# sjy-dv/coltt

Measured on AMD Instinct MI355X. Metric: queries/sec @ recall@10, 10Mx768 HNSW, higher is better.
Workload: dtype f32

## Files before the change

coltt_amd/csrc/pq.hip:

```cpp
#include <algorithm>
#include <atomic>
#include <type_traits>

#include "common.hpp"
#include "exact.hpp"
#include "select.hpp"

using namespace coltt;
using namespace coltt::dev;

namespace {

typedef float f32x2 __attribute__((ext_vector_type(2)));
constexpr int PQ_LDS_MAX = 152 * 1024;

template <int KIND, int LEN = 0>
__device__ __forceinline__ float pq_dist(const float* __restrict__ x, const float* __restrict__ y, int len_rt) {
  const int len = LEN > 0 ? LEN : len_rt;
  float acc[32];
#pragma unroll
  for (int u = 0; u < 32; u++) acc[u] = 0.f;
#define PQ_BLOCK_(I_)                                                                                   \
  _Pragma("unroll") for (int u = 0; u < 32; u++) {                                                      \
    const float xv = x[(I_) + u], yv = y[(I_) + u];                                                     \
// ... 121 lines not shown
}

__global__ void pq_place_codes_kernel(const uint8_t* __restrict__ src, uint64_t n, int m, int C, const uint32_t* __restrict__ slots, uint64_t slot_base,
                                      uint8_t* __restrict__ codes, int T, int PB, uint32_t* __restrict__ bad) {
  const uint64_t t = (uint64_t)blockIdx.x * blockDim.x + threadIdx.x;
  if (t >= n * (uint64_t)m) return;
  const uint64_t i = t / m; const int j = (int)(t - i * m);
  const uint8_t c = src[t];
  if ((int)c >= C) { atomicAdd(bad, 1u); return; }
  codes[code_offset(slots ? slots[i] : slot_base + i, j, T, PB)] = c;
}
__global__ void pq_fetch_codes_kernel(const uint8_t* __restrict__ codes, int T, int PB, uint64_t first, uint64_t n, int m, uint8_t* __restrict__ out) {
  const uint64_t t = (uint64_t)blockIdx.x * blockDim.x + threadIdx.x;
  if (t >= n * (uint64_t)m) return;
  const uint64_t i = t / m; const int j = (int)(t - i * m);
  out[t] = codes[code_offset(first + i, j, T, PB)];
}
__global__ void pq_move_row_kernel(uint8_t* __restrict__ codes, int T, int PB, int mp, uint64_t dst, uint64_t src) {
  const int j = (int)(blockIdx.x * blockDim.x + threadIdx.x);
  if (j < mp) codes[code_offset(dst, j, T, PB)] = codes[code_offset(src, j, T, PB)];
}

__global__ void pq_train_init_kernel(const float* __restrict__ vecs, int m, int C, int dsub, float* __restrict__ cb) {
  const uint64_t t = (uint64_t)blockIdx.x * blockDim.x + threadIdx.x;
  if (t >= (uint64_t)m * C * dsub) return;
  const int e = (int)(t % dsub); const int c = (int)((t / dsub) % C); const int j = (int)(t / ((uint64_t)dsub * C));
  cb[t] = vecs[((size_t)c * m + j) * dsub + e];
}
__global__ void pq_train_update_kernel(const float* __restrict__ vecs, uint64_t n, int m, int C, int dsub, const uint8_t* __restrict__ codes,
                                       int T, int PB, float* __restrict__ cb) {
  const uint64_t t = (uint64_t)blockIdx.x * blockDim.x + threadIdx.x;
  if (t >= (uint64_t)m * C * dsub) return;
  const int e = (int)(t % dsub); const int c = (int)((t / dsub) % C); const int j = (int)(t / ((uint64_t)dsub * C));
  float s = 0.f; uint32_t cnt = 0;
  for (uint64_t i = 0; i < n; i++) {
    if (codes[code_offset(i, j, T, PB)] != (uint8_t)c) continue;
    s += vecs[(i * (uint64_t)m + j) * dsub + e];
    cnt++;
  }
  if (cnt) cb[t] = div_rn(s, (float)cnt);
}

template <int W> struct PqRaw;
template <> struct PqRaw<1> { typedef uint32_t type; };
template <> struct PqRaw<2> { typedef u32x2e type; };
template <> struct PqRaw<4> { typedef u32x4e type; };
template <int W> __device__ __forceinline__ uint32_t pq_word(const typename PqRaw<W>::type& r, int i) {
  if constexpr (W == 1) return r;
  else if constexpr (W == 2) return i == 0 ? r.x : r.y;
  else return i == 0 ? r.x : (i == 1 ? r.y : (i == 2 ? r.z : r.w));
}

constexpr int PQ_RING = 8;

template <int W, int QB>
__global__ __launch_bounds__(1024) void pq_scan_kernel(const uint8_t* __restrict__ codes, int T, int mp, const float* __restrict__ lut_g, int nq,
                                                       uint64_t begin, uint64_t end, const uint32_t* __restrict__ thr,
                                                       unsigned long long* __restrict__ cand, uint32_t* __restrict__ cnt, uint32_t cap) {
  extern __shared__ __attribute__((aligned(16))) float lut[];
  typedef typename PqRaw<W>::type raw_t;
  const int tid = threadIdx.x, lane = tid & 63;
  const int q0 = (int)blockIdx.y * QB;
  const size_t lq = (size_t)mp * 256;
  if constexpr (QB == 1) {
    const f32x4* src = reinterpret_cast<const f32x4*>(lut_g + (size_t)q0 * lq);
    f32x4* dst = reinterpret_cast<f32x4*>(lut);
    for (int i = tid; i < mp * 64; i += blockDim.x) dst[i] = src[i];
  } else if constexpr (QB == 2) {
    for (int i = tid; i < mp * 256; i += blockDim.x) {
      f32x2 v;
      v.x = lut_g[(size_t)q0 * lq + i];
      v.y = q0 + 1 < nq ? lut_g[(size_t)(q0 + 1) * lq + i] : 0.f;
      reinterpret_cast<f32x2*>(lut)[i] = v;
    }
  } else {
    for (int i = tid; i < mp * 256; i += blockDim.x) {
      f32x4 v;
      v.x = lut_g[(size_t)q0 * lq + i];
      v.y = q0 + 1 < nq ? lut_g[(size_t)(q0 + 1) * lq + i] : 0.f;
      v.z = q0 + 2 < nq ? lut_g[(size_t)(q0 + 2) * lq + i] : 0.f;
      v.w = q0 + 3 < nq ? lut_g[(size_t)(q0 + 3) * lq + i] : 0.f;
      reinterpret_cast<f32x4*>(lut)[i] = v;
    }
  }
  uint32_t th[QB]; bool qv[QB];
#pragma unroll
  for (int q = 0; q < QB; q++) { qv[q] = q0 + q < nq; th[q] = qv[q] ? thr[q0 + q] : 0u; }
  __syncthreads();

  const int wave = __builtin_amdgcn_readfirstlane(tid >> 6);
  const int wpb = (int)(blockDim.x >> 6);
  const uint64_t tile_end = (end + 63) >> 6;
  const uint64_t tstride = (uint64_t)gridDim.x * wpb;
  uint64_t ptile = (begin >> 6) + (uint64_t)blockIdx.x * wpb + wave, ctile = ptile;
  int pt = 0, ct = 0;
  if (ctile >= tile_end) return;
  constexpr int PBYTES = 4 * W;
#define PQ_LOAD(dst)                                                                                                      \
  {                                                                                                                       \
    const uint64_t lt_ = ptile < tile_end ? ptile : tile_end - 1;                                                         \
    dst = *reinterpret_cast<const raw_t*>(codes + ((lt_ * (uint64_t)T + (uint64_t)pt) * 64 + (uint64_t)lane) * PBYTES);   \
    if (++pt == T) { pt = 0; ptile += tstride; }                                                                          \
  }
  constexpr int R = W == 4 ? PQ_RING : 2 * PQ_RING;
  raw_t cur[R], nxt[R];
#pragma unroll
  for (int u = 0; u < R; u++) PQ_LOAD(cur[u])
  typedef typename std::conditional<QB == 1, float, typename std::conditional<QB == 2, f32x2, f32x4>::type>::type acc_t;
  acc_t acc;
  if constexpr (QB == 1) acc = 0.f; else if constexpr (QB == 2) acc = f32x2{0.f, 0.f}; else acc = f32x4{0.f, 0.f, 0.f, 0.f};
  while (ctile < tile_end) {
#pragma unroll
    for (int u = 0; u < R; u++) PQ_LOAD(nxt[u])
#pragma unroll
    for (int u = 0; u < R; u++) {
      const raw_t raw = cur[u];
      const float* lp = lut + (size_t)ct * (PBYTES * 256 * QB);
#pragma unroll
      for (int d = 0; d < W; d++) {
        const uint32_t wd = pq_word<W>(raw, d);
#pragma unroll
        for (int b = 0; b < 4; b++) {
          const uint32_t code = (wd >> (8 * b)) & 0xffu;
          if constexpr (QB == 1) acc = acc + lp[(d * 4 + b) * 256 + code];
          else if constexpr (QB == 2) acc = acc + *reinterpret_cast<const f32x2*>(lp + ((size_t)(d * 4 + b) * 256 + code) * 2);
          else acc = acc + *reinterpret_cast<const f32x4*>(lp + ((size_t)(d * 4 + b) * 256 + code) * 4);
        }
      }
      if (++ct == T) {
        const uint64_t row = (ctile << 6) + (uint64_t)lane;
        const bool valid = ctile < tile_end && row >= begin && row < end;
#pragma unroll
        for (int q = 0; q < QB; q++) {
          float sc;
          if constexpr (QB == 1) sc = acc; else if constexpr (QB == 2) sc = q == 0 ? acc.x : acc.y; else sc = q == 0 ? acc.x : (q == 1 ? acc.y : (q == 2 ? acc.z : acc.w));
          const uint32_t key = score_key(sc);
          if (valid && qv[q] && key <= th[q]) {
            const uint32_t idx = atomicAdd(&cnt[q0 + q], 1u);
            if (idx < cap) cand[(size_t)(q0 + q) * cap + idx] = ((unsigned long long)key << 32) | (uint32_t)row;
          }
        }
        if constexpr (QB == 1) acc = 0.f; else if constexpr (QB == 2) acc = f32x2{0.f, 0.f}; else acc = f32x4{0.f, 0.f, 0.f, 0.f};
        ct = 0; ctile += tstride;
      }
    }
#pragma unroll
    for (int u = 0; u < R; u++) cur[u] = nxt[u];
  }
#undef PQ_LOAD
}

constexpr uint32_t PQ1_KMAX = 64;
constexpr uint32_t PQ1_WL = 128;
static __device__ __forceinline__ void pq_wave_sync() {
  __builtin_amdgcn_fence(__ATOMIC_RELEASE, "wavefront");
  __builtin_amdgcn_wave_barrier();
  __builtin_amdgcn_fence(__ATOMIC_ACQUIRE, "wavefront");
}
static __device__ __forceinline__ uint32_t pq1_compress(unsigned long long* __restrict__ wl, uint32_t nl, uint32_t k, uint32_t& thw, int lane, uint32_t* __restrict__ ovf) {
  const bool h0 = (uint32_t)lane < nl, h1 = 64u + (uint32_t)lane < nl;
  const unsigned long long e0 = h0 ? wl[lane] : ~0ull, e1 = h1 ? wl[64 + lane] : ~0ull;
  uint32_t r0 = 0, r1 = 0;
  for (uint32_t j = 0; j < nl; j++) { const unsigned long long ej = wl[j]; r0 += ej < e0 ? 1u : 0u; r1 += ej < e1 ? 1u : 0u; }
  const unsigned long long m0 = __ballot(h0 && r0 == k - 1), m1 = __ballot(h1 && r1 == k - 1);
  const uint32_t kth = m0 ? (uint32_t)__builtin_amdgcn_readlane((int)(uint32_t)(e0 >> 32), __builtin_ctzll(m0))
                          : (uint32_t)__builtin_amdgcn_readlane((int)(uint32_t)(e1 >> 32), __builtin_ctzll(m1 | (1ull << 63)));
  const bool k0 = h0 && (uint32_t)(e0 >> 32) <= kth, k1 = h1 && (uint32_t)(e1 >> 32) <= kth;
  const unsigned long long b0 = __ballot(k0), b1 = __ballot(k1), lt = (1ull << lane) - 1ull;
  const uint32_t n0 = (uint32_t)__popcll(b0), p1 = n0 + (uint32_t)__popcll(b1 & lt), tot = n0 + (uint32_t)__popcll(b1);
  pq_wave_sync();
  if (k0) wl[__popcll(b0 & lt)] = e0;
  if (k1 && p1 < PQ1_WL) wl[p1] = e1;
  pq_wave_sync();
  thw = kth;
  if (tot > 64u) { if (lane == 0) atomicOr(ovf, 1u); return 64u; }
  return tot;
}

template <int W>
__global__ __launch_bounds__(1024) void pq_scan1_kernel(const uint8_t* __restrict__ codes, int T, int mp, const float* __restrict__ lut_g, uint64_t end, uint32_t k,
                                                        unsigned long long* __restrict__ cand, uint32_t* __restrict__ cnt, uint32_t cap, uint32_t* __restrict__ ovf) {
  extern __shared__ __attribute__((aligned(16))) float lut[];
  __shared__ uint32_t s_wn[16], s_kth;
  typedef typename PqRaw<W>::type raw_t;
  const int tid = threadIdx.x, lane = tid & 63;
  const int wave = __builtin_amdgcn_readfirstlane(tid >> 6);
  const int wpb = (int)(blockDim.x >> 6);
  unsigned long long* const wl = reinterpret_cast<unsigned long long*>(lut + (size_t)mp * 256) + (size_t)wave * PQ1_WL;
  unsigned long long* const bl = reinterpret_cast<unsigned long long*>(lut + (size_t)mp * 256) + (size_t)wpb * PQ1_WL;
  {
    const f32x4* src = reinterpret_cast<const f32x4*>(lut_g);
    f32x4* dst = reinterpret_cast<f32x4*>(lut);
    for (int i = tid; i < mp * 64; i += blockDim.x) dst[i] = src[i];
  }
  if (tid == 0) s_kth = 0xffffffffu;
  __syncthreads();
  const uint64_t tile_end = (end + 63) >> 6;
  const uint64_t tstride = (uint64_t)gridDim.x * wpb;
  uint64_t ptile = (uint64_t)blockIdx.x * wpb + wave, ctile = ptile;
  int pt = 0, ct = 0;
  uint32_t nl = 0, thw = 0xffffffffu;
  const unsigned long long ltm = (1ull << lane) - 1ull;
  constexpr int PBYTES = 4 * W;
#define PQ_LOAD(dst)                                                                                                      \
  {                                                                                                                       \
    const uint64_t lt_ = ptile < tile_end ? ptile : tile_end - 1;                                                         \
    dst = *reinterpret_cast<const raw_t*>(codes + ((lt_ * (uint64_t)T + (uint64_t)pt) * 64 + (uint64_t)lane) * PBYTES);   \
    if (++pt == T) { pt = 0; ptile += tstride; }                                                                          \
  }
  constexpr int R = W == 4 ? PQ_RING : 2 * PQ_RING;
  if (ctile < tile_end) {
    raw_t cur[R], nxt[R];
#pragma unroll
    for (int u = 0; u < R; u++) PQ_LOAD(cur[u])
    float acc = 0.f;
    while (ctile < tile_end) {
#pragma unroll
      for (int u = 0; u < R; u++) PQ_LOAD(nxt[u])
#pragma unroll
      for (int u = 0; u < R; u++) {
        const raw_t raw = cur[u];
        const float* lp = lut + (size_t)ct * (PBYTES * 256);
#pragma unroll
        for (int d = 0; d < W; d++) {
          const uint32_t wd = pq_word<W>(raw, d);
#pragma unroll
          for (int b = 0; b < 4; b++) acc = acc + lp[(d * 4 + b) * 256 + ((wd >> (8 * b)) & 0xffu)];
        }
        if (++ct == T) {
          const uint64_t row = (ctile << 6) + (uint64_t)lane;
          const uint32_t key = score_key(acc);
          const bool pass = ctile < tile_end && row < end && key <= thw;
          const unsigned long long pm = __ballot(pass);
          if (pm) {
            if (pass) wl[nl + (uint32_t)__popcll(pm & ltm)] = ((unsigned long long)key << 32) | (uint32_t)row;
            nl += (uint32_t)__popcll(pm);
            pq_wave_sync();
            if (nl > 64u) nl = pq1_compress(wl, nl, k, thw, lane, ovf);
          }
          acc = 0.f; ct = 0; ctile += tstride;
        }
      }
#pragma unroll
      for (int u = 0; u < R; u++) cur[u] = nxt[u];
    }
    if (nl > k) nl = pq1_compress(wl, nl, k, thw, lane, ovf);
  }
#undef PQ_LOAD
  if (lane == 0) s_wn[wave] = nl;
  __syncthreads();
  uint32_t base = 0, tot = 0;
  for (int w = 0; w < wpb; w++) { const uint32_t c = s_wn[w]; base += w < wave ? c : 0u; tot += c; }
  for (uint32_t i = lane; i < nl; i += 64) bl[base + i] = wl[i];
  __syncthreads();
  if (tot >= k) {
    for (uint32_t i = tid; i < tot; i += blockDim.x) {
      const unsigned long long e = bl[i];
      uint32_t rank = 0;
      for (uint32_t j = 0; j < tot; j++) rank += bl[j] < e ? 1u : 0u;
      if (rank == k - 1) s_kth = (uint32_t)(e >> 32);
    }
    __syncthreads();
  }
  const uint32_t kth = s_kth;
  for (uint32_t i = tid; i < tot; i += blockDim.x) {
    const unsigned long long e = bl[i];
    if ((uint32_t)(e >> 32) > kth) continue;
    const uint32_t idx = atomicAdd(&cnt[0], 1u);
    if (idx < cap) cand[idx] = e;
  }
}

__global__ __launch_bounds__(256) void pq_scan_global_kernel(const uint8_t* __restrict__ codes, int T, int PB, int m, int mp, const float* __restrict__ lut_g,
                                                             uint64_t begin, uint64_t end, const uint32_t* __restrict__ thr,
                                                             unsigned long long* __restrict__ cand, uint32_t* __restrict__ cnt, uint32_t cap) {
  const int q = blockIdx.y;
  const float* lut = lut_g + (size_t)q * mp * 256;
  const uint32_t th = thr[q];
  for (uint64_t row = begin + (uint64_t)blockIdx.x * blockDim.x + threadIdx.x; row < end; row += (uint64_t)gridDim.x * blockDim.x) {
    float acc = 0.f;
    for (int j = 0; j < m; j++) acc = acc + lut[(size_t)j * 256 + codes[code_offset(row, j, T, PB)]];
    const uint32_t key = score_key(acc);
    if (key <= th) {
      const uint32_t idx = atomicAdd(&cnt[q], 1u);
      if (idx < cap) cand[(size_t)q * cap + idx] = ((unsigned long long)key << 32) | (uint32_t)row;
    }
  }
}

__global__ void pq_init_kernel(uint32_t* cnt, uint32_t* thr, uint32_t* ovf, int nq) {
  const int q = blockIdx.x * blockDim.x + threadIdx.x;
  if (q < nq) { cnt[q] = 0; thr[q] = 0xffffffffu; }
  if (q == 0) *ovf = 0;
}

struct PCtx {
  hipStream_t stream = nullptr;
  hipEvent_t ev0 = nullptr, ev1 = nullptr, evs0 = nullptr, evs1 = nullptr;
  DevBuf w_q, w_lut, w_cand, w_cnt, w_out_ids, w_out_sc, w_out_cnt;
  int init() {
    COLTT_HIP(hipStreamCreateWithFlags(&stream, hipStreamNonBlocking));
    COLTT_HIP(hipEventCreate(&ev0)); COLTT_HIP(hipEventCreate(&ev1));
    COLTT_HIP(hipEventCreate(&evs0)); COLTT_HIP(hipEventCreate(&evs1));
    return COLTT_OK;
  }
  ~PCtx() {
    for (hipEvent_t e : {ev0, ev1, evs0, evs1}) if (e) (void)hipEventDestroy(e);
    if (stream) (void)hipStreamDestroy(stream);
  }
};

struct Pq : Object {
  uint32_t dim = 0, m = 0, C = 0, dsub = 0; int metric = 0;
  int mp = 0, PB = 0, T = 0;
  bool trained = false;
  uint64_t n = 0, cap = 0;
  DevBuf cb, codes, ids;
  bool dense = true; uint64_t dense_base = 0;
  std::unordered_map<uint64_t, uint32_t> id2slot; std::vector<uint64_t> h_ids;
  hipStream_t stream = nullptr;
  DevBuf w_raw, w_slots, w_bad;
  std::atomic<float> last_ms{0.f}, last_scan_ms{0.f};
  std::atomic<uint64_t> last_scan_rows{0};
  CtxPool<PCtx> pool;
  ~Pq() override { (void)hipSetDevice(device); if (stream) (void)hipStreamDestroy(stream); }
  size_t tile_bytes() const { return (size_t)64 * mp; }
  int reserve(uint64_t rows) {
    if (rows <= cap) return COLTT_OK;
    uint64_t nc = std::max<uint64_t>({rows, cap + cap / 2, 1024});
    nc = (nc + 63) & ~63ull;
    const size_t old = codes.cap;
    COLTT_TRY(codes.reserve(nc / 64 * tile_bytes(), true, stream));
    if (codes.cap > old) {
      COLTT_HIP(hipMemsetAsync(codes.as<uint8_t>() + old, 0, codes.cap - old, stream));
      COLTT_HIP(hipStreamSynchronize(stream));
    }
    if (!dense) COLTT_TRY(ids.reserve(nc * 8, true, stream));
    cap = nc;
    return COLTT_OK;
  }
  int undense() {
    if (!dense) return COLTT_OK;
    h_ids.resize(n); id2slot.reserve(n * 2);
    for (uint64_t s = 0; s < n; s++) { h_ids[s] = dense_base + s; id2slot[dense_base + s] = (uint32_t)s; }
    dense = false;
    COLTT_TRY(ids.reserve(std::max<uint64_t>(cap, 1024) * 8, false, stream));
    if (n) COLTT_HIP(hipMemcpyAsync(ids.p, h_ids.data(), n * 8, hipMemcpyHostToDevice, stream));
    COLTT_HIP(hipStreamSynchronize(stream));
    return COLTT_OK;
  }
};

struct PqPlan { std::vector<uint32_t> slots; std::vector<uint64_t> new_ids; uint64_t nn = 0; };
int plan_upsert(const Pq* p, const uint64_t* ids, uint64_t first_id, size_t n, PqPlan& pl) {
  pl.slots.resize(n); pl.nn = p->n;
  std::unordered_map<uint64_t, uint32_t> fresh;
  for (size_t i = 0; i < n; i++) {
    const uint64_t id = ids ? ids[i] : first_id + i;
    auto it = p->id2slot.find(id);
    if (it != p->id2slot.end()) { pl.slots[i] = it->second; continue; }
    auto r = fresh.emplace(id, (uint32_t)pl.nn);
    if (r.second) { pl.new_ids.push_back(id); pl.nn++; }
    pl.slots[i] = r.first->second;
  }
  if (pl.nn > 0xffffffffull) return fail(COLTT_E_UNSUPPORTED, "pq upsert: more than 2^32-1 rows in one store");
  return COLTT_OK;
}
void last_wins(const PqPlan& pl, size_t n, std::vector<size_t>& keep) {
  std::unordered_map<uint32_t, size_t> last;
  for (size_t i = 0; i < n; i++) last[pl.slots[i]] = i;
  keep.clear();
  if (last.size() == n) return;
  for (size_t i = 0; i < n; i++) if (last[pl.slots[i]] == i) keep.push_back(i);
}
void commit_upsert(Pq* p, const PqPlan& pl) {
  for (size_t j = 0; j < pl.new_ids.size(); j++) { p->id2slot[pl.new_ids[j]] = (uint32_t)(p->n + j); p->h_ids.push_back(pl.new_ids[j]); }
  p->n = pl.nn;
}

int launch_encode(Pq* p, hipStream_t s, const float* d_vecs, uint64_t n, const uint32_t* d_slots, uint64_t slot_base, uint8_t* codes) {
  if (n == 0) return COLTT_OK;
  const size_t cb_bytes = (size_t)p->C * p->dsub * 4;
  const int lds_cb = cb_bytes <= 64 * 1024;
  const size_t lds = lds_cb ? cb_bytes : 0;
  dim3 grid(ceil_div(n, 256), p->m);
#define PQ_ENC(DS)                                                                                                               \
  {                                                                                                                              \
    auto kern = pq_encode_kernel<DS>;                                                                                            \
    if (lds > 48 * 1024) COLTT_HIP(hipFuncSetAttribute(reinterpret_cast<const void*>(kern), hipFuncAttributeMaxDynamicSharedMemorySize, (int)lds)); \
    kern<<<grid, 256, lds, s>>>(p->cb.as<float>(), (int)p->m, (int)p->C, (int)p->dsub, d_vecs, n, d_slots, slot_base, lds_cb, codes, p->T, p->PB); \
  }
  switch (p->dsub) {
    case 4: PQ_ENC(4) break;
    case 8: PQ_ENC(8) break;
    case 12: PQ_ENC(12) break;
    case 16: PQ_ENC(16) break;
    case 24: PQ_ENC(24) break;
    case 32: PQ_ENC(32) break;
    default: PQ_ENC(0) break;
  }
#undef PQ_ENC
  COLTT_HIP(hipGetLastError());
  return COLTT_OK;
}

template <int W>
int launch_scan_w(Pq* p, PCtx* c, int QBq, uint64_t b, uint64_t e, int nq, const float* lut, const uint32_t* thr, unsigned long long* cand, uint32_t* cnt, uint32_t cap) {
  const size_t lds = (size_t)p->mp * 1024 * QBq;
  const int threads = lds > 80 * 1024 ? 1024 : (lds > 40 * 1024 ? 512 : 256);
  const int wpb = threads / 64;
  const int blocks_per_cu = std::max<int>(1, std::min<int>(2048 / threads, (int)((160 * 1024) / std::max<size_t>(lds, 1))));
  const uint64_t tiles = ((e + 63) >> 6) - (b >> 6);
  const uint32_t gx = (uint32_t)std::max<uint64_t>(1, std::min<uint64_t>((tiles + wpb - 1) / wpb, (uint64_t)256 * blocks_per_cu));
  dim3 grid(gx, (nq + QBq - 1) / QBq);
  if (QBq == 1) {
    auto kern = pq_scan_kernel<W, 1>;
    COLTT_HIP(hipFuncSetAttribute(reinterpret_cast<const void*>(kern), hipFuncAttributeMaxDynamicSharedMemorySize, (int)std::max<size_t>(lds, 1024)));
    kern<<<grid, threads, lds, c->stream>>>(p->codes.as<uint8_t>(), p->T, p->mp, lut, nq, b, e, thr, cand, cnt, cap);
  } else if (QBq == 2) {
    auto kern = pq_scan_kernel<W, 2>;
    COLTT_HIP(hipFuncSetAttribute(reinterpret_cast<const void*>(kern), hipFuncAttributeMaxDynamicSharedMemorySize, (int)std::max<size_t>(lds, 1024)));
    kern<<<grid, threads, lds, c->stream>>>(p->codes.as<uint8_t>(), p->T, p->mp, lut, nq, b, e, thr, cand, cnt, cap);
  } else {
    auto kern = pq_scan_kernel<W, 4>;
    COLTT_HIP(hipFuncSetAttribute(reinterpret_cast<const void*>(kern), hipFuncAttributeMaxDynamicSharedMemorySize, (int)std::max<size_t>(lds, 1024)));
    kern<<<grid, threads, lds, c->stream>>>(p->codes.as<uint8_t>(), p->T, p->mp, lut, nq, b, e, thr, cand, cnt, cap);
  }
  COLTT_HIP(hipGetLastError());
  return COLTT_OK;
}

int launch_scan(Pq* p, PCtx* c, uint64_t b, uint64_t e, int nq, const float* lut, const uint32_t* thr, unsigned long long* cand, uint32_t* cnt, uint32_t cap) {
  const size_t one = (size_t)p->mp * 1024;
  if (one > (size_t)PQ_LDS_MAX) {
    dim3 grid((uint32_t)std::min<uint64_t>(ceil_div(e - b, 256), 256 * 8), nq);
    pq_scan_global_kernel<<<grid, 256, 0, c->stream>>>(p->codes.as<uint8_t>(), p->T, p->PB, (int)p->m, p->mp, lut, b, e, thr, cand, cnt, cap);
    COLTT_HIP(hipGetLastError());
    return COLTT_OK;
  }
  const int QBq = nq < 2 ? 1 : (one * 4 <= (size_t)PQ_LDS_MAX ? 4 : (one * 2 <= (size_t)PQ_LDS_MAX ? 2 : 1));
  if (p->PB == 16) return launch_scan_w<4>(p, c, QBq, b, e, nq, lut, thr, cand, cnt, cap);
  if (p->PB == 8) return launch_scan_w<2>(p, c, QBq, b, e, nq, lut, thr, cand, cnt, cap);
  return launch_scan_w<1>(p, c, QBq, b, e, nq, lut, thr, cand, cnt, cap);
}

bool scan1_geometry(const Pq* p, uint32_t k, int* threads_out, size_t* lds_out) {
  const char* e = getenv("COLTT_PQ_ONE");
  const bool off = e && e[0] == '0';
  if (off || k > PQ1_KMAX) return false;
  const size_t table = (size_t)p->mp * 1024;
  const int threads = table > 80 * 1024 ? 1024 : (table > 40 * 1024 ? 512 : 256);
  const size_t lds = table + (size_t)(threads / 64) * (PQ1_WL + 64) * 8;
  if (lds > (size_t)PQ_LDS_MAX) return false;
  *threads_out = threads; *lds_out = lds;
  return true;
}
template <int W>
int launch_scan1_w(Pq* p, PCtx* c, int threads, size_t lds, uint64_t total, uint32_t k, const float* lut, unsigned long long* cand, uint32_t* cnt, uint32_t cap, uint32_t* ovf) {
  const int wpb = threads / 64;
  const int blocks_per_cu = std::max<int>(1, std::min<int>(2048 / threads, (int)((160 * 1024) / lds)));
  const uint64_t tiles = (total + 63) >> 6;
  const uint32_t gx = (uint32_t)std::max<uint64_t>(1, std::min<uint64_t>((tiles + wpb - 1) / wpb, (uint64_t)256 * blocks_per_cu));
  auto kern = pq_scan1_kernel<W>;
  COLTT_HIP(hipFuncSetAttribute(reinterpret_cast<const void*>(kern), hipFuncAttributeMaxDynamicSharedMemorySize, (int)lds));
  kern<<<gx, threads, lds, c->stream>>>(p->codes.as<uint8_t>(), p->T, p->mp, lut, total, k, cand, cnt, cap, ovf);
  COLTT_HIP(hipGetLastError());
  return COLTT_OK;
}

constexpr size_t PQ_GROUP = 256;
int pq_search_group(Pq* p, PCtx* c, const float* queries, bool q_on_device, size_t nq, uint32_t k, uint64_t* out_ids, float* out_scores,
                    uint32_t* out_counts, bool out_on_device, float* acc_ms) {
  const float* d_q = queries;
  if (!q_on_device) {
    COLTT_TRY(c->w_q.reserve(nq * p->dim * 4));
    COLTT_HIP(hipMemcpyAsync(c->w_q.p, queries, nq * p->dim * 4, hipMemcpyHostToDevice, c->stream));
    d_q = c->w_q.as<float>();
  }
  uint64_t* d_oi = out_ids; float* d_os = out_scores; uint32_t* d_oc = out_counts;
  if (!out_on_device) {
    COLTT_TRY(c->w_out_ids.reserve(nq * k * 8)); COLTT_TRY(c->w_out_sc.reserve(nq * k * 4)); COLTT_TRY(c->w_out_cnt.reserve(nq * 4));
    d_oi = c->w_out_ids.as<uint64_t>(); d_os = c->w_out_sc.as<float>(); d_oc = c->w_out_cnt.as<uint32_t>();
  }
  const uint32_t cap = std::max<uint32_t>(65536u, 8u * k);
  COLTT_TRY(c->w_lut.reserve(nq * (size_t)p->mp * 256 * 4));
  COLTT_TRY(c->w_cand.reserve(nq * (size_t)cap * 8));
  COLTT_TRY(c->w_cnt.reserve((2 * nq + 4) * 4));
  uint32_t* cnt = c->w_cnt.as<uint32_t>(); uint32_t* thr = cnt + nq; uint32_t* ovf = thr + nq;
  unsigned long long* cand = c->w_cand.as<unsigned long long>();
  float* lut = c->w_lut.as<float>();
  const uint64_t* ids = p->dense ? nullptr : p->ids.as<uint64_t>();
  const uint64_t total = p->n;
  COLTT_HIP(hipEventRecord(c->ev0, c->stream));
  {
    dim3 grid(p->mp, (uint32_t)nq);
    if (p->metric == COLTT_PQ_COSINE) pq_lut_kernel<0><<<grid, 256, 0, c->stream>>>(p->cb.as<float>(), (int)p->m, (int)p->C, (int)p->dsub, d_q, p->mp, lut, cnt, thr, ovf);
    else if (p->metric == COLTT_PQ_EUCLIDEAN) pq_lut_kernel<1><<<grid, 256, 0, c->stream>>>(p->cb.as<float>(), (int)p->m, (int)p->C, (int)p->dsub, d_q, p->mp, lut, cnt, thr, ovf);
    else pq_lut_kernel<2><<<grid, 256, 0, c->stream>>>(p->cb.as<float>(), (int)p->m, (int)p->C, (int)p->dsub, d_q, p->mp, lut, cnt, thr, ovf);
  }
  bool timed_scan = false;
  auto scan = [&](uint64_t b, uint64_t e, bool big) -> int {
    if (big) COLTT_HIP(hipEventRecord(c->evs0, c->stream));
    COLTT_TRY(launch_scan(p, c, b, e, (int)nq, lut, thr, cand, cnt, cap));
    if (big) { COLTT_HIP(hipEventRecord(c->evs1, c->stream)); timed_scan = true; p->last_scan_rows.store(e - b); }
    flat_select_kernel<<<(uint32_t)nq, 256, 0, c->stream>>>(cand, cnt, thr, cap, k, 1, ids, p->dense_base, ovf, d_oi, d_os, d_oc);
    return COLTT_OK;
  };
  int t1 = 0; size_t lds1 = 0;
  if (total == 0) {
    flat_select_kernel<<<(uint32_t)nq, 256, 0, c->stream>>>(cand, cnt, thr, cap, k, 1, ids, p->dense_base, ovf, d_oi, d_os, d_oc);
  } else if (nq == 1 && total > 65536 && scan1_geometry(p, k, &t1, &lds1)) {
    COLTT_HIP(hipEventRecord(c->evs0, c->stream));
    if (p->PB == 16) COLTT_TRY(launch_scan1_w<4>(p, c, t1, lds1, total, k, lut, cand, cnt, cap, ovf));
    else if (p->PB == 8) COLTT_TRY(launch_scan1_w<2>(p, c, t1, lds1, total, k, lut, cand, cnt, cap, ovf));
    else COLTT_TRY(launch_scan1_w<1>(p, c, t1, lds1, total, k, lut, cand, cnt, cap, ovf));
    COLTT_HIP(hipEventRecord(c->evs1, c->stream)); timed_scan = true; p->last_scan_rows.store(total);
    flat_select_kernel<<<1, 256, 0, c->stream>>>(cand, cnt, thr, cap, k, 1, ids, p->dense_base, ovf, d_oi, d_os, d_oc);
  } else {
    uint64_t s0 = std::min<uint64_t>({total, (uint64_t)cap, (std::max<uint64_t>(4096, 4ull * k) + 63) & ~63ull});
    for (uint64_t b = 0, e = s0; b < total; b = e, e = std::min<uint64_t>(total, e * 64)) COLTT_TRY(scan(b, e, e == total));
  }
  auto fetch = [&](uint32_t* h_ovf) -> int {
    COLTT_HIP(hipEventRecord(c->ev1, c->stream));
    COLTT_HIP(hipGetLastError());
    COLTT_HIP(hipMemcpyAsync(h_ovf, ovf, 4, hipMemcpyDeviceToHost, c->stream));
    if (!out_on_device) {
      COLTT_HIP(hipMemcpyAsync(out_ids, d_oi, nq * k * 8, hipMemcpyDeviceToHost, c->stream));
      COLTT_HIP(hipMemcpyAsync(out_scores, d_os, nq * k * 4, hipMemcpyDeviceToHost, c->stream));
      COLTT_HIP(hipMemcpyAsync(out_counts, d_oc, nq * 4, hipMemcpyDeviceToHost, c->stream));
    }
    COLTT_HIP(hipStreamSynchronize(c->stream));
    return COLTT_OK;
  };
  uint32_t h_ovf = 0;
  COLTT_TRY(fetch(&h_ovf));
  if (h_ovf && total) {
    pq_init_kernel<<<ceil_div(nq, 256), 256, 0, c->stream>>>(cnt, thr, ovf, (int)nq);
    const uint64_t seg = (cap - std::min<uint32_t>(k, cap / 2)) & ~63ull;
    for (uint64_t b = 0; b < total; b += seg) COLTT_TRY(scan(b, std::min<uint64_t>(total, b + seg), false));
    COLTT_TRY(fetch(&h_ovf));
  }
  float ms = 0.f;
  (void)hipEventElapsedTime(&ms, c->ev0, c->ev1);
  if (acc_ms) *acc_ms += ms;
  if (timed_scan) { float sms = 0.f; (void)hipEventElapsedTime(&sms, c->evs0, c->evs1); p->last_scan_ms.store(sms); }
  return COLTT_OK;
}

int pq_search_common(Pq* p, PCtx* c, const float* queries, bool q_on_device, size_t nq, uint32_t k, uint64_t* out_ids, float* out_scores,
                     uint32_t* out_counts, bool out_on_device) {
  if (k == 0 || k > K_MAX) return fail(COLTT_E_UNSUPPORTED, "pq search: k=%u outside [1,%u]", k, K_MAX);
  if (nq == 0) return COLTT_OK;
  if (!p->trained) return fail(COLTT_E_INVALID, "pq search: the quantiser has no codebooks yet (coltt_pq_set_codebooks / coltt_pq_train)");
  float total_ms = 0.f;
  for (size_t q0 = 0; q0 < nq; q0 += PQ_GROUP) {
    const size_t gn = std::min(PQ_GROUP, nq - q0);
    COLTT_TRY(pq_search_group(p, c, queries + q0 * p->dim, q_on_device, gn, k, out_ids + q0 * k, out_scores + q0 * k, out_counts + q0, out_on_device, &total_ms));
  }
  p->last_ms.store(total_ms);
  return COLTT_OK;
}

}

int coltt::pq_snapshot(coltt_handle_t h, PqShape* shape, DevBuf* cb_out, hipStream_t s) {
  auto p = lookup<Pq>(h);
  if (!p) return fail(COLTT_E_NOT_FOUND, "pq snapshot: unknown quantiser handle");
  ReadLock g(p->rw);
  if (!p->trained) return fail(COLTT_E_INVALID, "pq snapshot: the quantiser has no codebooks yet (coltt_pq_set_codebooks / coltt_pq_train)");
  shape->dim = p->dim; shape->m = p->m; shape->C = p->C; shape->dsub = p->dsub; shape->metric = p->metric;
  const size_t bytes = (size_t)p->m * p->C * p->dsub * 4;
  COLTT_TRY(cb_out->reserve(bytes));
  COLTT_HIP(hipMemcpyAsync(cb_out->p, p->cb.p, bytes, hipMemcpyDefault, s));
  COLTT_HIP(hipStreamSynchronize(s));
  return COLTT_OK;
}

int coltt::pq_encode_rowmajor(hipStream_t s, const float* d_cb, const PqShape& sh, const float* d_vecs, uint64_t n, uint8_t* d_codes, uint32_t row_bytes) {
  if (n == 0) return COLTT_OK;
  const size_t cb_bytes = (size_t)sh.C * sh.dsub * 4;
  const int lds_cb = cb_bytes <= 64 * 1024;
  const size_t lds = lds_cb ? cb_bytes : 0;
  dim3 grid(ceil_div(n, 256), sh.m);
#define PQ_ENC(DS)                                                                                                               \
  {                                                                                                                              \
    auto kern = pq_encode_kernel<DS>;                                                                                            \
    if (lds > 48 * 1024) COLTT_HIP(hipFuncSetAttribute(reinterpret_cast<const void*>(kern), hipFuncAttributeMaxDynamicSharedMemorySize, (int)lds)); \
    kern<<<grid, 256, lds, s>>>(d_cb, (int)sh.m, (int)sh.C, (int)sh.dsub, d_vecs, n, nullptr, 0, lds_cb, d_codes, 1, (int)row_bytes);    \
  }
  switch (sh.dsub) {
    case 4: PQ_ENC(4) break;
    case 8: PQ_ENC(8) break;
    case 12: PQ_ENC(12) break;
    case 16: PQ_ENC(16) break;
    case 24: PQ_ENC(24) break;
    case 32: PQ_ENC(32) break;
    default: PQ_ENC(0) break;
  }
#undef PQ_ENC
  COLTT_HIP(hipGetLastError());
  return COLTT_OK;
}

int coltt::pq_lut16_batch(hipStream_t s, const float* d_cb, const PqShape& sh, const float* d_queries, size_t nq, uint32_t mp, uint32_t shift, uint32_t* d_qmax, unsigned short* d_lut) {
  if (nq == 0) return COLTT_OK;
  if (shift < 4 || shift > 8 || (1u << shift) < sh.C) return fail(COLTT_E_INVALID, "pq_lut16: %u centroids do not fit rows of %u entries", sh.C, 1u << shift);
  dim3 grid(ceil_div(mp, 256u >> shift), (uint32_t)nq);
  COLTT_HIP(hipMemsetAsync(d_qmax, 0, nq * 4, s));
#define COLTT_L16(K)                                                                                                                        \
  do {                                                                                                                                      \
    pq_lut16_max_kernel<K><<<grid, 256, 0, s>>>(d_cb, (int)sh.m, (int)sh.C, (int)sh.dsub, d_queries, (int)mp, (int)shift, d_qmax);          \
    pq_lut16_kernel<K><<<grid, 256, 0, s>>>(d_cb, (int)sh.m, (int)sh.C, (int)sh.dsub, d_queries, (int)mp, (int)shift, d_qmax, d_lut);        \
  } while (0)
  if (sh.metric == COLTT_PQ_COSINE) COLTT_L16(0);
  else if (sh.metric == COLTT_PQ_EUCLIDEAN) COLTT_L16(1);
  else COLTT_L16(2);
#undef COLTT_L16
  COLTT_HIP(hipGetLastError());
  return COLTT_OK;
}
int coltt::pq_centroid_norm_max(hipStream_t s, const float* d_cb, const PqShape& sh, uint32_t* d_scratch, float* out) {
  COLTT_HIP(hipMemsetAsync(d_scratch, 0, 4, s));
  const uint32_t nc = sh.m * sh.C;
  pq_centroid_norm_max_kernel<<<ceil_div(nc, 256u), 256, 0, s>>>(d_cb, nc, (int)sh.dsub, d_scratch);
  COLTT_HIP(hipGetLastError());
  uint32_t bits = 0;
  COLTT_HIP(hipMemcpyAsync(&bits, d_scratch, 4, hipMemcpyDeviceToHost, s));
  COLTT_HIP(hipStreamSynchronize(s));
  std::memcpy(out, &bits, 4);
  return COLTT_OK;
}

extern "C" {

int coltt_pq_create(uint32_t dim, int metric, uint32_t num_subvectors, uint32_t num_centroids, coltt_handle_t* out) {
  if (!out) return fail(COLTT_E_INVALID, "pq_create: out is NULL");
  if (metric != COLTT_PQ_COSINE && metric != COLTT_PQ_EUCLIDEAN && metric != COLTT_PQ_DOT) return fail(COLTT_E_INVALID, "pq_create: bad metric %d", metric);
  if (num_centroids < 2 || num_centroids > 256) return fail(COLTT_E_INVALID, "pq_create: numCentroids %u outside [2,256]", num_centroids);
  if (num_subvectors < 2) return fail(COLTT_E_INVALID, "pq_create: numSubVectors %u < 2", num_subvectors);
  if (dim == 0 || dim % num_subvectors) return fail(COLTT_E_INVALID, "pq_create: dim %u is not a multiple of numSubVectors %u", dim, num_subvectors);
  if (num_subvectors > 4096) return fail(COLTT_E_UNSUPPORTED, "pq_create: numSubVectors %u > 4096", num_subvectors);
  COLTT_DEVICE(-1);
  auto p = std::make_shared<Pq>();
  p->dim = dim; p->metric = metric; p->m = num_subvectors; p->C = num_centroids; p->dsub = dim / num_subvectors;
  p->mp = (int)((num_subvectors + 3) & ~3u);
  p->PB = p->mp % 16 == 0 ? 16 : (p->mp % 8 == 0 ? 8 : 4);
  p->T = p->mp / p->PB;
  p->device = coltt_dev_scope_.device();
  COLTT_HIP(hipStreamCreateWithFlags(&p->stream, hipStreamNonBlocking));
  COLTT_TRY(p->cb.reserve((size_t)p->m * p->C * p->dsub * 4));
  COLTT_TRY(p->w_bad.reserve(16));
  *out = Registry::get().add(p);
  return COLTT_OK;
}

int coltt_pq_destroy(coltt_handle_t h) {
  if (!Registry::get().erase(h)) return fail(COLTT_E_NOT_FOUND, "pq_destroy: unknown handle");
  return COLTT_OK;
}

int coltt_pq_set_codebooks(coltt_handle_t h, const float* codebooks) {
  auto p = lookup<Pq>(h);
  if (!p) return fail(COLTT_E_NOT_FOUND, "pq_set_codebooks: unknown handle");
  if (!codebooks) return fail(COLTT_E_INVALID, "pq_set_codebooks: NULL codebooks");
  WriteLock g(p->rw);
  COLTT_DEVICE(p->device);
  if (p->n) return fail(COLTT_E_INVALID, "pq_set_codebooks: the store holds %llu encoded rows — their codes belong to the current codebooks", (unsigned long long)p->n);
  COLTT_HIP(hipMemcpyAsync(p->cb.p, codebooks, (size_t)p->m * p->C * p->dsub * 4, hipMemcpyHostToDevice, p->stream));
  COLTT_HIP(hipStreamSynchronize(p->stream));
  p->trained = true;
// ... 254 lines not shown
```

coltt_amd/csrc/select.hpp:

```cpp
#pragma once
#include "exact.hpp"

namespace coltt {
namespace dev {

constexpr uint32_t K_MAX = 2048;
constexpr uint32_t SELECT_SMALL = 512;

static __device__ __forceinline__ uint64_t slot_id(const uint64_t* ids, uint64_t dense_base, uint32_t slot) {
  return ids ? ids[slot] : dense_base + slot;
}

typedef uint32_t sel_u32x4 __attribute__((ext_vector_type(4)));
typedef unsigned long long sel_u64x2 __attribute__((ext_vector_type(2)));
static __device__ __forceinline__ uint32_t sel_rank(const uint32_t* __restrict__ keys, const uint64_t* __restrict__ ids, uint32_t n4, uint32_t ki, uint64_t ii) {
  uint32_t rank = 0;
  for (uint32_t j = 0; j < n4; j += 4) {
    const sel_u32x4 kj = *reinterpret_cast<const sel_u32x4*>(keys + j);
    const sel_u64x2 ia = *reinterpret_cast<const sel_u64x2*>(ids + j), ib = *reinterpret_cast<const sel_u64x2*>(ids + j + 2);
    rank += ((kj.x < ki) || (kj.x == ki && ia.x < ii)) ? 1u : 0u;
    rank += ((kj.y < ki) || (kj.y == ki && ia.y < ii)) ? 1u : 0u;
    rank += ((kj.z < ki) || (kj.z == ki && ib.x < ii)) ? 1u : 0u;
    rank += ((kj.w < ki) || (kj.w == ki && ib.y < ii)) ? 1u : 0u;
  }
  return rank;
}

static __device__ __forceinline__ void sel_find_digit(const uint32_t* __restrict__ hist, uint32_t need, uint32_t* __restrict__ wave_tot,
                                                      uint32_t* __restrict__ s_digit, uint32_t* __restrict__ s_need) {
  const int tid = threadIdx.x, lane = tid & 63, wave = tid >> 6;
  const uint32_t h = hist[tid];
  uint32_t inc = h;
#pragma unroll
  for (int d = 1; d < 64; d <<= 1) {
    const uint32_t up = (uint32_t)__shfl_up((int)inc, d, 64);
    if (lane >= d) inc += up;
  }
  if (lane == 63) wave_tot[wave] = inc;
  __syncthreads();
  uint32_t base = 0;
  for (int w = 0; w < wave; w++) base += wave_tot[w];
  inc += base;
  const uint32_t exc = inc - h;
  if (exc < need && need <= inc) { *s_digit = (uint32_t)tid; *s_need = need - exc; }
}

template <uint32_t KCAP = K_MAX>
static __device__ __forceinline__ void flat_select_block(
    const int q, unsigned long long* __restrict__ cand_all, uint32_t* __restrict__ cnt_all, uint32_t* __restrict__ thr_all,
    uint32_t cap, uint32_t k, int nearest, const uint64_t* __restrict__ ids, uint64_t dense_base,
    uint32_t* __restrict__ overflow, uint64_t* __restrict__ out_ids, float* __restrict__ out_scores,
    uint32_t* __restrict__ out_counts) {
  static_assert(KCAP >= SELECT_SMALL, "the short-list path keeps every candidate in LDS");
  __shared__ uint32_t hist[256];
  __shared__ __attribute__((aligned(16))) uint32_t sel_key[KCAP + 4];
  __shared__ uint32_t sel_slot[KCAP];
  __shared__ __attribute__((aligned(16))) uint64_t sel_id[KCAP + 4];
  __shared__ uint32_t s_digit, s_need, s_nsel, s_wtot[4];
  const int tid = threadIdx.x;
  unsigned long long* cand = cand_all + (size_t)q * cap;
  uint32_t c = cnt_all[q];
  if (c > cap) { if (tid == 0) atomicOr(overflow, 1u); c = cap; }
  const uint32_t kk = k < c ? k : c;
  if (kk == 0) {
    if (tid == 0) { out_counts[q] = 0; cnt_all[q] = 0; thr_all[q] = nearest ? 0xffffffffu : 0u; }
    return;
  }
  const uint32_t flip = nearest ? 0u : 0xffffffffu;
  if (c <= SELECT_SMALL) {
    const uint64_t idflip_s = nearest ? 0ull : ~0ull;
    for (uint32_t i = tid; i < c; i += 256) {
      const unsigned long long e = cand[i];
      sel_key[i] = (uint32_t)(e >> 32) ^ flip; sel_slot[i] = (uint32_t)e; sel_id[i] = slot_id(ids, dense_base, (uint32_t)e) ^ idflip_s;
    }
    const uint32_t c4 = (c + 3u) & ~3u;
    if (tid < c4 - c) { sel_key[c + tid] = 0xffffffffu; sel_id[c + tid] = ~0ull; }
    __syncthreads();
    for (uint32_t i = tid; i < c; i += 256) {
      const uint32_t ki = sel_key[i]; const uint64_t ii = sel_id[i];
      const uint32_t rank = sel_rank(sel_key, sel_id, c4, ki, ii);
      if (rank >= kk) continue;
      const uint32_t pos = nearest ? rank : (kk - 1 - rank);
      const uint32_t key = ki ^ flip;
      out_ids[(size_t)q * k + pos] = ii ^ idflip_s;
      out_scores[(size_t)q * k + pos] = key_score(key);
      cand[pos] = ((unsigned long long)key << 32) | sel_slot[i];
      if (rank == kk - 1) thr_all[q] = (kk == k) ? key : (nearest ? 0xffffffffu : 0u);
    }
    if (tid == 0) { out_counts[q] = kk; cnt_all[q] = kk; }
    return;
  }
  uint32_t prefix = 0, mask = 0, need = kk;
  for (int pass = 3; pass >= 0; pass--) {
    const int shift = pass * 8;
    hist[tid] = 0;
    __syncthreads();
    for (uint32_t i = tid; i < c; i += 256) {
      uint32_t kp = (uint32_t)(cand[i] >> 32) ^ flip;
      if ((kp & mask) == prefix) atomicAdd(&hist[(kp >> shift) & 255u], 1u);
    }
    __syncthreads();
    sel_find_digit(hist, need, s_wtot, &s_digit, &s_need);
    __syncthreads();
    prefix |= s_digit << shift; mask |= 255u << shift; need = s_need;
    __syncthreads();
  }
  const uint32_t T = prefix;
  const uint32_t ties = hist[s_digit];
  const uint64_t idflip = nearest ? 0ull : ~0ull;
  uint64_t idT = ~0ull;
  if (ties > need) {
    uint64_t ipre = 0, imask = 0; uint32_t ineed = need;
    for (int pass = 7; pass >= 0; pass--) {
      const int shift = pass * 8;
      __syncthreads();
      hist[tid] = 0;
      __syncthreads();
      for (uint32_t i = tid; i < c; i += 256) {
        unsigned long long e = cand[i];
        if (((uint32_t)(e >> 32) ^ flip) != T) continue;
        uint64_t ip = slot_id(ids, dense_base, (uint32_t)e) ^ idflip;
        if ((ip & imask) == ipre) atomicAdd(&hist[(ip >> shift) & 255ull], 1u);
      }
      __syncthreads();
      sel_find_digit(hist, ineed, s_wtot, &s_digit, &s_need);
      __syncthreads();
      ipre |= (uint64_t)s_digit << shift; imask |= 255ull << shift; ineed = s_need;
    }
    idT = ipre;
  }
  if (tid == 0) s_nsel = 0;
  __syncthreads();
  for (uint32_t i = tid; i < c; i += 256) {
    unsigned long long e = cand[i];
    uint32_t kp = (uint32_t)(e >> 32) ^ flip;
    if (kp > T) continue;
    uint64_t ip = slot_id(ids, dense_base, (uint32_t)e) ^ idflip;
    if (kp == T && ip > idT) continue;
    uint32_t j = atomicAdd(&s_nsel, 1u);
    if (j < KCAP) { sel_key[j] = kp; sel_slot[j] = (uint32_t)e; sel_id[j] = ip; }
  }
  __syncthreads();
  const uint32_t ns = s_nsel < kk ? s_nsel : kk;
  const uint32_t ns4 = (ns + 3u) & ~3u;
  if (tid < ns4 - ns) { sel_key[ns + tid] = 0xffffffffu; sel_id[ns + tid] = ~0ull; }
  __syncthreads();
  for (uint32_t i = tid; i < ns; i += 256) {
    uint32_t ki = sel_key[i]; uint64_t ii = sel_id[i];
    const uint32_t rank = sel_rank(sel_key, sel_id, ns4, ki, ii);
    uint32_t pos = nearest ? rank : (ns - 1 - rank);
    uint32_t key = ki ^ flip;
    out_ids[(size_t)q * k + pos] = ii ^ idflip;
    out_scores[(size_t)q * k + pos] = key_score(key);
    cand[pos] = ((unsigned long long)key << 32) | sel_slot[i];
  }
  if (tid == 0) {
    out_counts[q] = ns; cnt_all[q] = ns;
    thr_all[q] = (ns == k) ? (T ^ flip) : (nearest ? 0xffffffffu : 0u);
  }
}

static __global__ __launch_bounds__(256) void flat_select_kernel(
    unsigned long long* __restrict__ cand_all, uint32_t* __restrict__ cnt_all, uint32_t* __restrict__ thr_all,
    uint32_t cap, uint32_t k, int nearest, const uint64_t* __restrict__ ids, uint64_t dense_base,
    uint32_t* __restrict__ overflow, uint64_t* __restrict__ out_ids, float* __restrict__ out_scores,
    uint32_t* __restrict__ out_counts) {
  flat_select_block<K_MAX>((int)blockIdx.x, cand_all, cnt_all, thr_all, cap, k, nearest, ids, dense_base, overflow, out_ids, out_scores, out_counts);
}

static __global__ void init_group_kernel(uint32_t* cnt, uint32_t* thr, uint32_t* overflow, int nearest) {
  int q = threadIdx.x;
  if (q < 256) { cnt[q] = 0; thr[q] = nearest ? 0xffffffffu : 0u; }
  if (q == 0) *overflow = 0;
}



}
}
```

Before: 1.125 million.

## Fuse final top-k selection into the single-query PQ scan kernel via last-block pattern

Each block of the single-query PQ scan now writes its surviving candidates and its best entry to a per-block global region. The last block to finish is detected with an atomic counter. That block derives a bound from the per-block minima, gathers only candidates under the bound, and runs the flat selection in-kernel over reused LDS. This removes the separate select kernel launch and the global atomic contention on one counter. The cost is a larger scratch buffer, a serialized tail in one block, and a grid capped at a maximum block count.

```diff
diff --git a/coltt_amd/csrc/pq.hip b/coltt_amd/csrc/pq.hip
--- a/coltt_amd/csrc/pq.hip
+++ b/coltt_amd/csrc/pq.hip
@@ -297,6 +297,8 @@
 
 constexpr uint32_t PQ1_KMAX = 64;
 constexpr uint32_t PQ1_WL = 128;
+constexpr uint32_t PQ1_MAX_BLOCKS = 2048;
+constexpr size_t PQ1_FUSE_ENTRIES = (size_t)256 * 2048 + 2 * PQ1_MAX_BLOCKS;
 static __device__ __forceinline__ void pq_wave_sync() {
   __builtin_amdgcn_fence(__ATOMIC_RELEASE, "wavefront");
   __builtin_amdgcn_wave_barrier();
@@ -322,11 +324,19 @@
   return tot;
 }
 
+constexpr int PQ1_OWN = PQ1_MAX_BLOCKS / 256;
+static __device__ __forceinline__ unsigned long long* fuse_region(unsigned long long* cand, uint32_t cap) { return cand + cap; }
+static __device__ __forceinline__ unsigned long long* fuse_best(unsigned long long* cand, uint32_t cap) {
+  return cand + cap + (size_t)gridDim.x * (blockDim.x + 1);
+}
 template <int W>
 __global__ __launch_bounds__(1024) void pq_scan1_kernel(const uint8_t* __restrict__ codes, int T, int mp, const float* __restrict__ lut_g, uint64_t end, uint32_t k,
-                                                        unsigned long long* __restrict__ cand, uint32_t* __restrict__ cnt, uint32_t cap, uint32_t* __restrict__ ovf) {
+                                                        unsigned long long* __restrict__ cand, uint32_t* __restrict__ cnt, uint32_t cap, uint32_t* __restrict__ ovf,
+                                                        int fuse, uint32_t* __restrict__ thr, const uint64_t* __restrict__ ids, uint64_t dense_base,
+                                                        uint64_t* __restrict__ out_ids, float* __restrict__ out_scores, uint32_t* __restrict__ out_counts) {
   extern __shared__ __attribute__((aligned(16))) float lut[];
-  __shared__ uint32_t s_wn[16], s_kth;
+  __shared__ unsigned long long s_best;
+  __shared__ uint32_t s_wn[16], s_kth, s_last, s_n, s_w;
   typedef typename PqRaw<W>::type raw_t;
   const int tid = threadIdx.x, lane = tid & 63;
   const int wave = __builtin_amdgcn_readfirstlane(tid >> 6);
@@ -338,7 +348,7 @@
     f32x4* dst = reinterpret_cast<f32x4*>(lut);
     for (int i = tid; i < mp * 64; i += blockDim.x) dst[i] = src[i];
   }
-  if (tid == 0) s_kth = 0xffffffffu;
+  if (tid == 0) { s_kth = 0xffffffffu; s_best = ~0ull; s_n = 0; s_w = 0; }
   __syncthreads();
   const uint64_t tile_end = (end + 63) >> 6;
   const uint64_t tstride = (uint64_t)gridDim.x * wpb;
@@ -408,12 +418,92 @@
     __syncthreads();
   }
   const uint32_t kth = s_kth;
+  if (!fuse) {
+    for (uint32_t i = tid; i < tot; i += blockDim.x) {
+      const unsigned long long e = bl[i];
+      if ((uint32_t)(e >> 32) > kth) continue;
+      const uint32_t idx = atomicAdd(&cnt[0], 1u);
+      if (idx < cap) cand[idx] = e;
+    }
+    return;
+  }
   for (uint32_t i = tid; i < tot; i += blockDim.x) {
     const unsigned long long e = bl[i];
     if ((uint32_t)(e >> 32) > kth) continue;
-    const uint32_t idx = atomicAdd(&cnt[0], 1u);
-    if (idx < cap) cand[idx] = e;
-  }
+    atomicAdd(&s_n, 1u);
+    atomicMin(&s_best, e);
+  }
+  __syncthreads();
+  const size_t rstride = (size_t)blockDim.x + 1;
+  unsigned long long* const region = fuse_region(cand, cap) + (size_t)blockIdx.x * rstride;
+  for (uint32_t i = tid; i < tot; i += blockDim.x) {
+    const unsigned long long e = bl[i];
+    if ((uint32_t)(e >> 32) > kth) continue;
+    const uint32_t j = atomicAdd(&s_w, 1u);
+    __hip_atomic_store(region + 1 + j, e, __ATOMIC_RELAXED, __HIP_MEMORY_SCOPE_AGENT);
+  }
+  if (tid == 0) {
+    __hip_atomic_store(region, (unsigned long long)s_n, __ATOMIC_RELAXED, __HIP_MEMORY_SCOPE_AGENT);
+    __hip_atomic_store(fuse_best(cand, cap) + blockIdx.x, s_best, __ATOMIC_RELAXED, __HIP_MEMORY_SCOPE_AGENT);
+  }
+  asm volatile("s_waitcnt vmcnt(0)" ::: "memory");
+  __builtin_amdgcn_fence(__ATOMIC_RELEASE, "workgroup");
+  __syncthreads();
+  if (tid == 0) s_last = atomicAdd(thr, 1u) == gridDim.x - 2u ? 1u : 0u;
+  __syncthreads();
+  if (!s_last || tid >= 256) return;
+  __builtin_amdgcn_fence(__ATOMIC_ACQUIRE, "agent");
+  uint32_t* const gmin = reinterpret_cast<uint32_t*>(lut);
+  uint32_t nb[PQ1_OWN];
+  {
+    unsigned long long mine = ~0ull;
+#pragma unroll
+    for (int u = 0; u < PQ1_OWN; u++) {
+      const uint32_t b = (uint32_t)tid + 256u * (uint32_t)u;
+      const bool have = b < gridDim.x;
+      const unsigned long long n = have ? __hip_atomic_load(fuse_region(cand, cap) + (size_t)b * rstride, __ATOMIC_RELAXED, __HIP_MEMORY_SCOPE_AGENT) : 0ull;
+      const unsigned long long e = have ? __hip_atomic_load(fuse_best(cand, cap) + b, __ATOMIC_RELAXED, __HIP_MEMORY_SCOPE_AGENT) : ~0ull;
+      nb[u] = n < (unsigned long long)blockDim.x ? (uint32_t)n : blockDim.x;
+      mine = e < mine ? e : mine;
+    }
+    gmin[tid] = (uint32_t)(mine >> 32);
+  }
+  if (tid == 0) s_n = 0;
+  __syncthreads();
+  {
+    const uint32_t mk = gmin[tid];
+    uint32_t rank = 0;
+    for (int j = 0; j < 256; j += 4) {
+      const sel_u32x4 o = *reinterpret_cast<const sel_u32x4*>(gmin + j);
+      rank += (o.x < mk || (o.x == mk && j < tid)) ? 1u : 0u;
+      rank += (o.y < mk || (o.y == mk && j + 1 < tid)) ? 1u : 0u;
+      rank += (o.z < mk || (o.z == mk && j + 2 < tid)) ? 1u : 0u;
+      rank += (o.w < mk || (o.w == mk && j + 3 < tid)) ? 1u : 0u;
+    }
+    if (rank == k - 1) s_kth = mk;
+  }
+  __syncthreads();
+  const uint32_t bound = s_kth;
+  constexpr int B = 16;
+#pragma unroll
+  for (int u = 0; u < PQ1_OWN; u++) {
+    const unsigned long long* src = fuse_region(cand, cap) + (size_t)((uint32_t)tid + 256u * (uint32_t)u) * rstride + 1;
+    for (uint32_t i0 = 0; i0 < nb[u]; i0 += B) {
+      unsigned long long e[B];
+#pragma unroll
+      for (int v = 0; v < B; v++) e[v] = i0 + v < nb[u] ? __hip_atomic_load(src + i0 + v, __ATOMIC_RELAXED, __HIP_MEMORY_SCOPE_AGENT) : ~0ull;
+#pragma unroll
+      for (int v = 0; v < B; v++) {
+        if (i0 + v >= nb[u] || (uint32_t)(e[v] >> 32) > bound) continue;
+        const uint32_t j = atomicAdd(&s_n, 1u);
+        if (j < cap) cand[j] = e[v];
+      }
+    }
+  }
+  __syncthreads();
+  if (tid == 0) cnt[0] = s_n;
+  __syncthreads();
+  flat_select_with<SELECT_SMALL>(select_lds_over<SELECT_SMALL>(lut), 0, cand, cnt, thr, cap, k, 1, ids, dense_base, ovf, out_ids, out_scores, out_counts);
 }
 
 __global__ __launch_bounds__(256) void pq_scan_global_kernel(const uint8_t* __restrict__ codes, int T, int PB, int m, int mp, const float* __restrict__ lut_g,
@@ -589,7 +679,7 @@
   return launch_scan_w<1>(p, c, QBq, b, e, nq, lut, thr, cand, cnt, cap);
 }
 
-bool scan1_geometry(const Pq* p, uint32_t k, int* threads_out, size_t* lds_out) {
+bool scan1_geometry(const Pq* p, uint32_t k, int* threads_out, size_t* lds_out, bool* fuse_out) {
   const char* e = getenv("COLTT_PQ_ONE");
   const bool off = e && e[0] == '0';
   if (off || k > PQ1_KMAX) return false;
@@ -597,18 +687,20 @@
   const int threads = table > 80 * 1024 ? 1024 : (table > 40 * 1024 ? 512 : 256);
   const size_t lds = table + (size_t)(threads / 64) * (PQ1_WL + 64) * 8;
   if (lds > (size_t)PQ_LDS_MAX) return false;
-  *threads_out = threads; *lds_out = lds;
+  static_assert(select_lds_bytes<SELECT_SMALL>() <= 4 * 1024 + 4 * (PQ1_WL + 64) * 8, "the selection's LDS lies over the smallest table and its lists");
+  *threads_out = threads; *lds_out = lds; *fuse_out = !(e && e[0] == '2');
   return true;
 }
 template <int W>
-int launch_scan1_w(Pq* p, PCtx* c, int threads, size_t lds, uint64_t total, uint32_t k, const float* lut, unsigned long long* cand, uint32_t* cnt, uint32_t cap, uint32_t* ovf) {
+int launch_scan1_w(Pq* p, PCtx* c, int threads, size_t lds, uint64_t total, uint32_t k, const float* lut, unsigned long long* cand, uint32_t* cnt, uint32_t cap, uint32_t* ovf,
+                   bool fuse, uint32_t* thr, const uint64_t* ids, uint64_t* d_oi, float* d_os, uint32_t* d_oc) {
   const int wpb = threads / 64;
   const int blocks_per_cu = std::max<int>(1, std::min<int>(2048 / threads, (int)((160 * 1024) / lds)));
   const uint64_t tiles = (total + 63) >> 6;
-  const uint32_t gx = (uint32_t)std::max<uint64_t>(1, std::min<uint64_t>((tiles + wpb - 1) / wpb, (uint64_t)256 * blocks_per_cu));
+  const uint32_t gx = (uint32_t)std::max<uint64_t>(1, std::min<uint64_t>({(tiles + wpb - 1) / wpb, (uint64_t)256 * blocks_per_cu, (uint64_t)PQ1_MAX_BLOCKS}));
   auto kern = pq_scan1_kernel<W>;
   COLTT_HIP(hipFuncSetAttribute(reinterpret_cast<const void*>(kern), hipFuncAttributeMaxDynamicSharedMemorySize, (int)lds));
-  kern<<<gx, threads, lds, c->stream>>>(p->codes.as<uint8_t>(), p->T, p->mp, lut, total, k, cand, cnt, cap, ovf);
+  kern<<<gx, threads, lds, c->stream>>>(p->codes.as<uint8_t>(), p->T, p->mp, lut, total, k, cand, cnt, cap, ovf, fuse ? 1 : 0, thr, ids, p->dense_base, d_oi, d_os, d_oc);
   COLTT_HIP(hipGetLastError());
   return COLTT_OK;
 }
@@ -629,7 +721,7 @@
   }
   const uint32_t cap = std::max<uint32_t>(65536u, 8u * k);
   COLTT_TRY(c->w_lut.reserve(nq * (size_t)p->mp * 256 * 4));
-  COLTT_TRY(c->w_cand.reserve(nq * (size_t)cap * 8));
+  COLTT_TRY(c->w_cand.reserve((nq * (size_t)cap + PQ1_FUSE_ENTRIES) * 8));
   COLTT_TRY(c->w_cnt.reserve((2 * nq + 4) * 4));
   uint32_t* cnt = c->w_cnt.as<uint32_t>(); uint32_t* thr = cnt + nq; uint32_t* ovf = thr + nq;
   unsigned long long* cand = c->w_cand.as<unsigned long long>();
@@ -651,16 +743,16 @@
     flat_select_kernel<<<(uint32_t)nq, 256, 0, c->stream>>>(cand, cnt, thr, cap, k, 1, ids, p->dense_base, ovf, d_oi, d_os, d_oc);
     return COLTT_OK;
   };
-  int t1 = 0; size_t lds1 = 0;
+  int t1 = 0; size_t lds1 = 0; bool fuse1 = false;
   if (total == 0) {
     flat_select_kernel<<<(uint32_t)nq, 256, 0, c->stream>>>(cand, cnt, thr, cap, k, 1, ids, p->dense_base, ovf, d_oi, d_os, d_oc);
-  } else if (nq == 1 && total > 65536 && scan1_geometry(p, k, &t1, &lds1)) {
+  } else if (nq == 1 && total > 65536 && scan1_geometry(p, k, &t1, &lds1, &fuse1)) {
     COLTT_HIP(hipEventRecord(c->evs0, c->stream));
-    if (p->PB == 16) COLTT_TRY(launch_scan1_w<4>(p, c, t1, lds1, total, k, lut, cand, cnt, cap, ovf));
-    else if (p->PB == 8) COLTT_TRY(launch_scan1_w<2>(p, c, t1, lds1, total, k, lut, cand, cnt, cap, ovf));
-    else COLTT_TRY(launch_scan1_w<1>(p, c, t1, lds1, total, k, lut, cand, cnt, cap, ovf));
+    if (p->PB == 16) COLTT_TRY(launch_scan1_w<4>(p, c, t1, lds1, total, k, lut, cand, cnt, cap, ovf, fuse1, thr, ids, d_oi, d_os, d_oc));
+    else if (p->PB == 8) COLTT_TRY(launch_scan1_w<2>(p, c, t1, lds1, total, k, lut, cand, cnt, cap, ovf, fuse1, thr, ids, d_oi, d_os, d_oc));
+    else COLTT_TRY(launch_scan1_w<1>(p, c, t1, lds1, total, k, lut, cand, cnt, cap, ovf, fuse1, thr, ids, d_oi, d_os, d_oc));
     COLTT_HIP(hipEventRecord(c->evs1, c->stream)); timed_scan = true; p->last_scan_rows.store(total);
-    flat_select_kernel<<<1, 256, 0, c->stream>>>(cand, cnt, thr, cap, k, 1, ids, p->dense_base, ovf, d_oi, d_os, d_oc);
+    if (!fuse1) flat_select_kernel<<<1, 256, 0, c->stream>>>(cand, cnt, thr, cap, k, 1, ids, p->dense_base, ovf, d_oi, d_os, d_oc);
   } else {
     uint64_t s0 = std::min<uint64_t>({total, (uint64_t)cap, (std::max<uint64_t>(4096, 4ull * k) + 63) & ~63ull});
     for (uint64_t b = 0, e = s0; b < total; b = e, e = std::min<uint64_t>(total, e * 64)) COLTT_TRY(scan(b, e, e == total));
diff --git a/coltt_amd/csrc/select.hpp b/coltt_amd/csrc/select.hpp
--- a/coltt_amd/csrc/select.hpp
+++ b/coltt_amd/csrc/select.hpp
@@ -45,18 +45,34 @@
   if (exc < need && need <= inc) { *s_digit = (uint32_t)tid; *s_need = need - exc; }
 }
 
-template <uint32_t KCAP = K_MAX>
-static __device__ __forceinline__ void flat_select_block(
+struct SelectLds {
+  uint32_t* hist;
+  uint32_t* sel_key;
+  uint32_t* sel_slot;
+  uint64_t* sel_id;
+  uint32_t *s_digit, *s_need, *s_nsel, *s_wtot;
+};
+template <uint32_t KCAP> constexpr size_t select_lds_bytes() { return (size_t)(KCAP + 4) * 8 + (size_t)(KCAP + 4) * 4 + (size_t)KCAP * 4 + 256 * 4 + 8 * 4; }
+template <uint32_t KCAP>
+static __device__ __forceinline__ SelectLds select_lds_over(void* base) {
+  uint64_t* const id = reinterpret_cast<uint64_t*>(base);
+  uint32_t* const key = reinterpret_cast<uint32_t*>(id + KCAP + 4);
+  uint32_t* const slot = key + KCAP + 4;
+  uint32_t* const hist = slot + KCAP;
+  uint32_t* const w = hist + 256;
+  return SelectLds{hist, key, slot, id, w, w + 1, w + 2, w + 4};
+}
+
+template <uint32_t KCAP>
+static __device__ __forceinline__ void flat_select_with(
+    const SelectLds& L,
     const int q, unsigned long long* __restrict__ cand_all, uint32_t* __restrict__ cnt_all, uint32_t* __restrict__ thr_all,
     uint32_t cap, uint32_t k, int nearest, const uint64_t* __restrict__ ids, uint64_t dense_base,
     uint32_t* __restrict__ overflow, uint64_t* __restrict__ out_ids, float* __restrict__ out_scores,
     uint32_t* __restrict__ out_counts) {
   static_assert(KCAP >= SELECT_SMALL, "the short-list path keeps every candidate in LDS");
-  __shared__ uint32_t hist[256];
-  __shared__ __attribute__((aligned(16))) uint32_t sel_key[KCAP + 4];
-  __shared__ uint32_t sel_slot[KCAP];
-  __shared__ __attribute__((aligned(16))) uint64_t sel_id[KCAP + 4];
-  __shared__ uint32_t s_digit, s_need, s_nsel, s_wtot[4];
+  uint32_t* const hist = L.hist; uint32_t* const sel_key = L.sel_key; uint32_t* const sel_slot = L.sel_slot; uint64_t* const sel_id = L.sel_id;
+  uint32_t& s_digit = *L.s_digit; uint32_t& s_need = *L.s_need; uint32_t& s_nsel = *L.s_nsel; uint32_t* const s_wtot = L.s_wtot;
   const int tid = threadIdx.x;
   unsigned long long* cand = cand_all + (size_t)q * cap;
   uint32_t c = cnt_all[q];
@@ -160,6 +176,21 @@
   }
 }
 
+template <uint32_t KCAP = K_MAX>
+static __device__ __forceinline__ void flat_select_block(
+    const int q, unsigned long long* __restrict__ cand_all, uint32_t* __restrict__ cnt_all, uint32_t* __restrict__ thr_all,
+    uint32_t cap, uint32_t k, int nearest, const uint64_t* __restrict__ ids, uint64_t dense_base,
+    uint32_t* __restrict__ overflow, uint64_t* __restrict__ out_ids, float* __restrict__ out_scores,
+    uint32_t* __restrict__ out_counts) {
+  __shared__ uint32_t hist[256];
+  __shared__ __attribute__((aligned(16))) uint32_t sel_key[KCAP + 4];
+  __shared__ uint32_t sel_slot[KCAP];
+  __shared__ __attribute__((aligned(16))) uint64_t sel_id[KCAP + 4];
+  __shared__ uint32_t s_digit, s_need, s_nsel, s_wtot[4];
+  const SelectLds L = {hist, sel_key, sel_slot, sel_id, &s_digit, &s_need, &s_nsel, s_wtot};
+  flat_select_with<KCAP>(L, q, cand_all, cnt_all, thr_all, cap, k, nearest, ids, dense_base, overflow, out_ids, out_scores, out_counts);
+}
+
 static __global__ __launch_bounds__(256) void flat_select_kernel(
     unsigned long long* __restrict__ cand_all, uint32_t* __restrict__ cnt_all, uint32_t* __restrict__ thr_all,
     uint32_t cap, uint32_t k, int nearest, const uint64_t* __restrict__ ids, uint64_t dense_base,
```

Result: slower. 1.103 million (-1.9%).
